# menezesandre/stackrl

Measured on AMD Instinct MI355X. Metric: env steps/sec (batched Stack-v0), higher is better.
Workload: dtype f32

## Files before the change

### stackrl_amd/csrc/settle.hip

```cpp
#include "srl_device.h"
#include "srl_kernels.h"
#include "stage.h"

#ifdef SRL_DIAG_JITTER
__device__ __forceinline__ void srl_jitter_sync() {
  unsigned t = (unsigned)__builtin_readcyclecounter() * 2654435761u + (threadIdx.x >> 6) * 40503u;
  t = __builtin_amdgcn_readfirstlane(t);
  const int n = (t >> 13) & 15;
  for (int i = 0; i < n; ++i) __builtin_amdgcn_s_sleep(16);
  __builtin_amdgcn_fence(__ATOMIC_RELEASE, "workgroup");
  __builtin_amdgcn_s_barrier();
  __builtin_amdgcn_fence(__ATOMIC_ACQUIRE, "workgroup");
  t = t * 1664525u + 1013904223u;
  const int m = (t >> 13) & 15;
  for (int i = 0; i < m; ++i) __builtin_amdgcn_s_sleep(16);
}
#define __syncthreads() srl_jitter_sync()
#endif

template <int T, int PP> struct Variant;

__device__ __forceinline__ int pair_word(int p) {
  int j = (int)((1.0f + sqrtf(1.0f + 8.0f * (float)p)) * 0.5f);
  while (j * (j - 1) / 2 > p) --j;
// ... 416 lines not shown
  const f2 d2 = F2(imp, imp);
#pragma unroll
  for (int c = 0; c < 3; ++c) { u.a[c] = fma2(r.ua[c], d2, u.a[c]); u.b[c] = fma2(r.ub[c], d2, u.b[c]); }
}

__device__ __forceinline__ float contact_target(const DevParams& P, float dist) {
  float inv_dt = 1.0f / P.c.sim_time_step;
  float pen = dist + P.c.linear_slop;
  return pen > 0.0f ? -(pen * inv_dt) : -((pen * P.c.erp) * inv_dt);
}

struct Point {
  PRow n, t1, t2;
  float target, in, i1, i2, ima, imb, mu;
  int a, b;
  int colour;
  int idx;
  bool valid;
};

struct GRow { v3 ca, aa; float rk, k; };
struct GPoint {
  GRow n, t1, t2;
  float target, in, i1, i2, ima, mu;
  int a, idx;
  bool valid;
};

__device__ __forceinline__ GRow make_grow(v3 d, v3 ra, float ima, const m3& Ia) {
  GRow r;
  r.ca = cross(ra, d);
  r.aa = mmul(Ia, r.ca);
  const float k = ima + dot(cross(r.aa, ra), d);
  r.rk = 1.0f / k;
  r.k = k;
  return r;
}

template <int AXIS, int SGN>
__device__ __forceinline__ void grow_solve(const GRow& r, float ima, v3& v, v3& w, float target, float& acc, float lo,
                                           float hi, float& res) {
  float& va = AXIS == 0 ? v.x : AXIS == 1 ? v.y : v.z;
  const float vrel = fmaf(r.ca.x, w.x, fmaf(r.ca.y, w.y, fmaf(r.ca.z, w.z, SGN < 0 ? -va : va)));
  float dl = fmaf(-vrel, r.rk, target * r.rk);
  const float na = __builtin_amdgcn_fmed3f(acc + dl, lo, hi);
  dl = na - acc;
  acc = na;
  res = fmaxf(res, fabsf(dl * r.k));
  va = fmaf(SGN < 0 ? -ima : ima, dl, va);
  w = madd(w, r.aa, dl);
}

template <int AXIS, int SGN>
__device__ __forceinline__ void grow_apply(const GRow& r, float ima, v3& v, v3& w, float imp) {
  float& va = AXIS == 0 ? v.x : AXIS == 1 ? v.y : v.z;
  va = fmaf(SGN < 0 ? -ima : ima, imp, va);
  w = madd(w, r.aa, imp);
}

__device__ __forceinline__ GPoint make_ground_point(const Lds& L, int b, int i) {
  const DevParams& P = *L.P;
  GPoint p;
  p.valid = false; p.a = b; p.idx = i;
  p.in = 0.0f; p.i1 = 0.0f; p.i2 = 0.0f; p.target = 0.0f; p.ima = 0.0f; p.mu = 0.0f;
  const float* g = L.GM(b);
  if (i >= __float_as_int(g[0])) return p;
  p.valid = true;
  p.ima = L.BC(b)[0];
  p.mu = P.c.friction_rock * P.c.friction_ground;
  const m3 Ia = ldm(L.IW(b));
  const int vid = __float_as_int(g[SRL_GM_VID + i]);
  const v3 pw = ld3(L.WV(b) + 3 * vid);
  const v3 ra = V(pw.x, pw.y, pw.z - P.c.collision_margin) - ld3(L.X(b));
  v3 n = V(0.0f, 0.0f, 1.0f), t1, t2;
  plane_space(n, t1, t2);
  p.n = make_grow(n, ra, p.ima, Ia);
  p.t1 = make_grow(t1, ra, p.ima, Ia);
  p.t2 = make_grow(t2, ra, p.ima, Ia);
  p.target = contact_target(P, g[SRL_GM_DIST + i]);
  p.in = g[SRL_GM_IN + i]; p.i1 = g[SRL_GM_T1 + i]; p.i2 = g[SRL_GM_T2 + i];
  return p;
}

template <bool WARM>
__device__ __forceinline__ void ground_turn(const Lds& L, GPoint& p, float& res) {
  const float ws = L.P->c.warmstart;
  v3 v, w;
  ldvw(L, p.a, v, w);
  if (WARM) {
    p.in = p.in * ws; p.i1 = p.i1 * ws; p.i2 = p.i2 * ws;
    grow_apply<2, 1>(p.n, p.ima, v, w, p.in);
    grow_apply<1, -1>(p.t1, p.ima, v, w, p.i1);
    grow_apply<0, 1>(p.t2, p.ima, v, w, p.i2);
  } else {
    grow_solve<2, 1>(p.n, p.ima, v, w, p.target, p.in, 0.0f, 1e30f, res);
    const float lim = p.mu * p.in;
    grow_solve<1, -1>(p.t1, p.ima, v, w, 0.0f, p.i1, -lim, lim, res);
    grow_solve<0, 1>(p.t2, p.ima, v, w, 0.0f, p.i2, -lim, lim, res);
  }
  stvw(L, p.a, v, w);
}

#define SRL_CG_WORDS 28
struct GBody {
  float acc[SRL_GMAXP][3];
  float ima;
  int np, b;
  float* pvw;
  const float4* rec;
};

__device__ __forceinline__ float4* cg_rec(const Lds& L, int b, int i) {
  return (float4*)L.WV(0) + (SRL_CG_WORDS / 4) * (SRL_GMAXP * b + i);
}
__device__ __forceinline__ void cg_store(const Lds& L, const GPoint& p) {
  float4* r = cg_rec(L, p.a, p.idx);
  r[0] = make_float4(p.n.ca.x, p.n.ca.y, p.n.ca.z, p.n.rk);
  r[1] = make_float4(p.n.aa.x, p.n.aa.y, p.n.aa.z, p.target * p.n.rk);
  r[2] = make_float4(p.t1.ca.x, p.t1.ca.y, p.t1.ca.z, p.t1.rk);
  r[3] = make_float4(p.t1.aa.x, p.t1.aa.y, p.t1.aa.z, p.n.k);
  r[4] = make_float4(p.t2.ca.x, p.t2.ca.y, p.t2.ca.z, p.t2.rk);
  r[5] = make_float4(p.t2.aa.x, p.t2.aa.y, p.t2.aa.z, p.t1.k);
  r[6] = make_float4(p.t2.k, p.mu, 0.0f * p.t1.rk, 0.0f * p.t2.rk);
}

template <int AXIS, int SGN>
__device__ __forceinline__ void grow_solve_t(v3 ca, v3 aa, float rk, float k, float ima, v3& v, v3& w, float trk, float& acc,
                                             float lo, float hi, float& res) {
  float& va = AXIS == 0 ? v.x : AXIS == 1 ? v.y : v.z;
  const float vrel = fmaf(ca.x, w.x, fmaf(ca.y, w.y, fmaf(ca.z, w.z, SGN < 0 ? -va : va)));
  float dl = fmaf(-vrel, rk, trk);
  const float na = __builtin_amdgcn_fmed3f(acc + dl, lo, hi);
  dl = na - acc;
  acc = na;
  res = fmaxf(res, fabsf(dl * k));
  va = fmaf(SGN < 0 ? -ima : ima, dl, va);
  w = madd(w, aa, dl);
}

struct GRec { f4 q[7]; };

template <bool WARM>
__device__ __forceinline__ void ground_point(const GRec& R, GBody& gb, int i, float ws, v3& v, v3& w, float& res) {
  const f4 q0 = R.q[0], q1 = R.q[1], q2 = R.q[2], q3 = R.q[3], q4 = R.q[4], q5 = R.q[5], q6 = R.q[6];
  if (WARM) {
    gb.acc[i][0] = gb.acc[i][0] * ws; gb.acc[i][1] = gb.acc[i][1] * ws; gb.acc[i][2] = gb.acc[i][2] * ws;
    GRow g; g.rk = 0.0f; g.k = 0.0f;
    g.ca = V(q0.x, q0.y, q0.z); g.aa = V(q1.x, q1.y, q1.z); grow_apply<2, 1>(g, gb.ima, v, w, gb.acc[i][0]);
    g.ca = V(q2.x, q2.y, q2.z); g.aa = V(q3.x, q3.y, q3.z); grow_apply<1, -1>(g, gb.ima, v, w, gb.acc[i][1]);
    g.ca = V(q4.x, q4.y, q4.z); g.aa = V(q5.x, q5.y, q5.z); grow_apply<0, 1>(g, gb.ima, v, w, gb.acc[i][2]);
  } else {
    grow_solve_t<2, 1>(V(q0.x, q0.y, q0.z), V(q1.x, q1.y, q1.z), q0.w, q3.w, gb.ima, v, w, q1.w, gb.acc[i][0], 0.0f, 1e30f, res);
    const float lim = q6.y * gb.acc[i][0];
    grow_solve_t<1, -1>(V(q2.x, q2.y, q2.z), V(q3.x, q3.y, q3.z), q2.w, q5.w, gb.ima, v, w, q6.z, gb.acc[i][1], -lim, lim, res);
    grow_solve_t<0, 1>(V(q4.x, q4.y, q4.z), V(q5.x, q5.y, q5.z), q4.w, q6.x, gb.ima, v, w, q6.w, gb.acc[i][2], -lim, lim, res);
  }
}

__device__ __forceinline__ GRec cg_load(const float4* rec, int i) {
  GRec R;
#pragma unroll
  for (int k = 0; k < 7; ++k) { const float4 t = rec[7 * i + k]; R.q[k].x = t.x; R.q[k].y = t.y; R.q[k].z = t.z; R.q[k].w = t.w; }
  return R;
}

template <int I>
__device__ __forceinline__ void cg_request(unsigned a, GRec& R, float& tie) {
  asm volatile(
      "ds_read_b128 %0, %8 offset:%9\n\tds_read_b128 %1, %8 offset:%10\n\tds_read_b128 %2, %8 offset:%11\n\t"
      "ds_read_b128 %3, %8 offset:%12\n\tds_read_b128 %4, %8 offset:%13\n\tds_read_b128 %5, %8 offset:%14\n\t"
      "ds_read_b128 %6, %8 offset:%15"
      : "=&v"(R.q[0]), "=&v"(R.q[1]), "=&v"(R.q[2]), "=&v"(R.q[3]), "=&v"(R.q[4]), "=&v"(R.q[5]), "=&v"(R.q[6]), "+v"(tie)
      : "v"(a), "n"(112 * I), "n"(112 * I + 16), "n"(112 * I + 32), "n"(112 * I + 48), "n"(112 * I + 64), "n"(112 * I + 80),
        "n"(112 * I + 96));
}
__device__ __forceinline__ void cg_request_first(unsigned avw, unsigned a, f4& a0, f2& a1, GRec& R) {
  asm volatile(
      "ds_read_b128 %0, %9\n\tds_read_b64 %1, %9 offset:16\n\t"
      "ds_read_b128 %2, %10\n\tds_read_b128 %3, %10 offset:16\n\tds_read_b128 %4, %10 offset:32\n\t"
      "ds_read_b128 %5, %10 offset:48\n\tds_read_b128 %6, %10 offset:64\n\tds_read_b128 %7, %10 offset:80\n\t"
      "ds_read_b128 %8, %10 offset:96"
      : "=&v"(a0), "=&v"(a1), "=&v"(R.q[0]), "=&v"(R.q[1]), "=&v"(R.q[2]), "=&v"(R.q[3]), "=&v"(R.q[4]), "=&v"(R.q[5]), "=&v"(R.q[6])
      : "v"(avw), "v"(a));
}
__device__ __forceinline__ void cg_arrive_first(f4& a0, f2& a1, GRec& R) {
  asm volatile("s_waitcnt lgkmcnt(7)"
               : "+v"(a0), "+v"(a1), "+v"(R.q[0]), "+v"(R.q[1]), "+v"(R.q[2]), "+v"(R.q[3]), "+v"(R.q[4]), "+v"(R.q[5]), "+v"(R.q[6]));
}
template <int LEFT>
__device__ __forceinline__ void cg_arrive(GRec& R, float& tie) {
  asm volatile("s_waitcnt lgkmcnt(%8)"
               : "+v"(R.q[0]), "+v"(R.q[1]), "+v"(R.q[2]), "+v"(R.q[3]), "+v"(R.q[4]), "+v"(R.q[5]), "+v"(R.q[6]), "+v"(tie)
               : "n"(LEFT));
}

template <bool WARM, bool AHEAD, bool KEEP>
__device__ __forceinline__ void ground_body(GBody& gb, float ws, v3& v, v3& w, float& res) {
  static_assert(SRL_CG_WORDS == 28, "cg_request reads seven float4 per record");
  const float4* rec = gb.rec;
  static_assert(SRL_GMAXP == 4, "four nested guards below");
  if (!AHEAD) {
    if (!KEEP) {
      const float4 a0 = *(const float4*)gb.pvw;
      const float2 a1 = *(const float2*)(gb.pvw + 4);
      v = V(a0.x, a0.z, a1.x); w = V(a0.y, a0.w, a1.y);
    }
    ground_point<WARM>(cg_load(rec, 0), gb, 0, ws, v, w, res);
    if (gb.np > 1) {
      ground_point<WARM>(cg_load(rec, 1), gb, 1, ws, v, w, res);
      if (gb.np > 2) {
        ground_point<WARM>(cg_load(rec, 2), gb, 2, ws, v, w, res);
        if (gb.np > 3) ground_point<WARM>(cg_load(rec, 3), gb, 3, ws, v, w, res);
      }
    }
  } else {
    const unsigned ra = (unsigned)(size_t)rec;
    GRec r0, r1, r2, r3;
    if (!KEEP) {
      f4 a0; f2 a1;
      float none = 0.0f;
      cg_request_first((unsigned)(size_t)gb.pvw, ra, a0, a1, r0);
      cg_request<1>(ra, r1, none);
      cg_arrive_first(a0, a1, r0);
      v = V(a0.x, a0.z, a1.x); w = V(a0.y, a0.w, a1.y);
    } else {
      cg_request<0>(ra, r0, w.z);
      cg_request<1>(ra, r1, w.z);
      cg_arrive<7>(r0, w.z);
    }
    ground_point<WARM>(r0, gb, 0, ws, v, w, res);
    cg_arrive<0>(r1, w.x);
    if (gb.np > 1) {
      cg_request<2>(ra, r2, w.z);
      ground_point<WARM>(r1, gb, 1, ws, v, w, res);
      cg_arrive<0>(r2, w.x);
      if (gb.np > 2) {
        cg_request<3>(ra, r3, w.z);
        ground_point<WARM>(r2, gb, 2, ws, v, w, res);
        cg_arrive<0>(r3, w.x);
        if (gb.np > 3) ground_point<WARM>(r3, gb, 3, ws, v, w, res);
      }
    }
  }
  if (!KEEP) { *(float4*)gb.pvw = make_float4(v.x, w.x, v.y, w.y); *(float2*)(gb.pvw + 4) = make_float2(v.z, w.z); }
}

__device__ __forceinline__ Point make_pair_point(const Lds& L, int sl, int i) {
  const DevParams& P = *L.P;
  Point p;
  p.valid = false; p.a = 0; p.b = 0; p.colour = 0; p.idx = i;
  p.in = 0.0f; p.i1 = 0.0f; p.i2 = 0.0f; p.target = 0.0f; p.ima = 0.0f; p.imb = 0.0f; p.mu = 0.0f;
  if (sl >= P.NS) return p;
  const int pid = L.POS()[sl];
  if (pid < 0) return p;
  const float* mp = L.MAN(sl);
  if (i >= __float_as_int(mp[0])) return p;
  p.valid = true;
  L.pair(pid, p.a, p.b);
  p.colour = L.COL()[sl];
  p.ima = L.BC(p.a)[0]; p.imb = L.BC(p.b)[0];
  p.mu = P.c.friction_rock * P.c.friction_rock;
  const float* q = mp + 4 + SRL_MP_WORDS * i;
  const m3 Ra = ldm(L.R(p.a)), Rb = ldm(L.R(p.b));
  const m3 Ia = ldm(L.IW(p.a)), Ib = ldm(L.IW(p.b));
  const v3 ra = mmul(Ra, ld3(q));
  const v3 rb = mmul(Rb, ld3(q + 3));
  v3 n = ld3(q + 6), t1, t2;
  plane_space(n, t1, t2);
  p.n = pack_row(make_row<true>(n, ra, rb, p.ima, Ia, p.imb, Ib), p.ima, p.imb);
  p.t1 = pack_row(make_row<true>(t1, ra, rb, p.ima, Ia, p.imb, Ib), p.ima, p.imb);
  p.t2 = pack_row(make_row<true>(t2, ra, rb, p.ima, Ia, p.imb, Ib), p.ima, p.imb);
  p.target = contact_target(P, q[9]);
  p.in = q[10]; p.i1 = q[11]; p.i2 = q[12];
  return p;
}

template <bool WARM>
__device__ __forceinline__ void point_turn(const Lds& L, Point& p, float& res) {
  const float ws = L.P->c.warmstart;
  Vel2 u;
  float* const pa = L.VW(p.a);
  float* const pb = L.VW(p.b);
  {
    const float4 a0 = *(const float4*)pa, b0 = *(const float4*)pb;
    const float2 a1 = *(const float2*)(pa + 4), b1 = *(const float2*)(pb + 4);
    u.a[0] = F2(a0.x, a0.y); u.a[1] = F2(a0.z, a0.w); u.a[2] = F2(a1.x, a1.y);
    u.b[0] = F2(b0.x, b0.y); u.b[1] = F2(b0.z, b0.w); u.b[2] = F2(b1.x, b1.y);
  }
  if (WARM) {
    p.in = p.in * ws; p.i1 = p.i1 * ws; p.i2 = p.i2 * ws;
    prow_apply(p.n, u, p.in);
    prow_apply(p.t1, u, p.i1);
    prow_apply(p.t2, u, p.i2);
  } else {
    prow_solve(p.n, u, p.target, p.in, 0.0f, 1e30f, res);
    const float lim = p.mu * p.in;
    prow_solve(p.t1, u, 0.0f, p.i1, -lim, lim, res);
    prow_solve(p.t2, u, 0.0f, p.i2, -lim, lim, res);
  }
  *(float4*)pa = make_float4(u.a[0].x, u.a[0].y, u.a[1].x, u.a[1].y); *(float2*)(pa + 4) = make_float2(u.a[2].x, u.a[2].y);
  *(float4*)pb = make_float4(u.b[0].x, u.b[0].y, u.b[1].x, u.b[1].y); *(float2*)(pb + 4) = make_float2(u.b[2].x, u.b[2].y);
}

template <bool WARM, int T, int PP, bool SOLO>
__device__ __forceinline__ bool solver_sweep(const Lds& L, GPoint& gp, GBody& gb, Point (&pp)[PP], int ncol, int gslot,
                                             const int (&pslot)[PP], int gsweep, const unsigned long long (&cm)[2]) {
  typedef Variant<T, PP> VA;
  static_assert(!SOLO || VA::SOLO, "a solo sweep in a variant that has none");
  float res = 0.0f;
  constexpr unsigned long long T0 = 0x1111111111111111ull;
  if (!VA::GROUND_BODY) {
    const unsigned long long gm = __ballot(gslot >= 0);
#pragma unroll
    for (int i = 0; i < SRL_GMAXP; ++i) {
      const unsigned long long t = gm & (T0 << i);
      if (t == 0) break;
      if (__builtin_amdgcn_inverse_ballot_w64(t)) ground_turn<WARM>(L, gp, res);
      __builtin_amdgcn_wave_barrier();
    }
  } else {
    v3 v, w;
    if (gb.np > 0) ground_body<WARM, !WARM && VA::GROUND_AHEAD, false>(gb, L.P->c.warmstart, v, w, res);
    __builtin_amdgcn_wave_barrier();
  }
  int c0 = 0;
  if (SOLO) {
#pragma unroll
    for (int c = 0; c < 2; ++c) {
      if (c >= ncol) break;
#pragma unroll
      for (int i = 0; i < 4; ++i) {
        const unsigned long long t = cm[c] & (T0 << i);
        if (t == 0) break;
        if (__builtin_amdgcn_inverse_ballot_w64(t)) point_turn<WARM>(L, pp[0], res);
        __builtin_amdgcn_wave_barrier();
      }
    }
    c0 = 2;
  }
#pragma unroll 1
  for (int c = c0; c < ncol; ++c) {
    if (!SOLO) __syncthreads();
    unsigned long long mc[PP];
#pragma unroll
    for (int r = 0; r < PP; ++r) mc[r] = __ballot((pslot[r] >> 2) == c);
#pragma unroll
    for (int i = 0; i < 4; ++i) {
      unsigned long long any = 0;
#pragma unroll
      for (int r = 0; r < PP; ++r) any |= mc[r] & (T0 << i);
      if (any == 0) break;
#pragma unroll
      for (int r = 0; r < PP; ++r)
        if (__builtin_amdgcn_inverse_ballot_w64(mc[r] & (T0 << i))) point_turn<WARM>(L, pp[r], res);
      __builtin_amdgcn_wave_barrier();
    }
  }
  if (SOLO) return WARM ? true : __ballot(res * res > L.P->c.residual_threshold) != 0ull;
  int* word = L.MISC() + M_RES0 + (gsweep & 1);
  if (!WARM) {
    if (__ballot(res * res > L.P->c.residual_threshold) != 0ull && (threadIdx.x & 63) == 0) *word = gsweep;
  }
  __syncthreads();
  return WARM ? true : *word == gsweep;
}

#ifdef SRL_STAMPS
#define STAMP(k) do { if (tid == 0) { long long _t = wall_clock64(); L.P->hdr[blockIdx.x].stamps[k] += _t - _t0; _t0 = _t; } } while (0)
#else
#define STAMP(k)
#endif

template <int T, int PP>
__device__ __forceinline__ void substep(const Lds& L, int nb, int tid, int& gsweep) {
  typedef Variant<T, PP> VA;
  const DevParams& P = *L.P;
  if (PP >= 2) asm volatile("" : "+v"(tid));
#ifdef SRL_STAMPS
  long long _t0 = wall_clock64();
#endif
  int* misc = L.MISC();
  if (tid < nb) body_frame(L, tid);
  if (tid == 0) { misc[M_FLAGS] = 0; misc[M_SOLO] = 1; }
  __syncthreads();
  STAMP(0);
  for (int it = tid; it < nb * P.VS; it += T) {
    const int b = it / P.VS, k = it - b * P.VS;
    if (k < __float_as_int(L.BC(b)[5])) {
      const m3 R = ldm(L.R(b));
      v3 lv;
      if (P.S_LV >= 0) lv = ld3(L.LV(b) + 3 * k);
      else { const float4 g4 = P.mv[__float_as_int(L.BC(b)[6]) + k]; lv = V(g4.x, g4.y, g4.z); }
      st3(L.WV(b) + 3 * k, mmul_add(R, lv, ld3(L.X(b))));
    }
  }
  __syncthreads();
  STAMP(1);
  for (int b = tid >> 4; b < nb; b += T >> 4) body_bounds_ground(L, b, tid & 15);
  __syncthreads();
  STAMP(2);
  const int npair = nb * (nb - 1) / 2;
  int fl = 0;
  for (int pid = tid; pid < npair; pid += T) {
    int i, j; L.pair(pid, i, j);
    v3 ai = ld3(L.AMIN(i)), bi = ld3(L.AMAX(i)), aj = ld3(L.AMIN(j)), bj = ld3(L.AMAX(j));
    bool ov = ai.x <= bj.x && aj.x <= bi.x && ai.y <= bj.y && aj.y <= bi.y && ai.z <= bj.z && aj.z <= bi.z;
    int sl = L.SOP()[pid];
    if (!ov && sl >= 0) { L.SOP()[pid] = -1; L.POS()[sl] = -1; fl |= 1; }
    if (ov && sl < 0) fl |= 2;
  }
  if (fl) atomicOr(&misc[M_FLAGS], fl);
  __syncthreads();
  const int flags = misc[M_FLAGS], ncol0 = misc[M_NCOL];
  if (flags || ncol0 < 0) {
    __syncthreads();
    if (tid == 0) {
      if (flags & 2) {
        for (int pid = 0; pid < npair; ++pid) {
          if (L.SOP()[pid] >= 0) continue;
          int i, j; L.pair(pid, i, j);
          v3 ai = ld3(L.AMIN(i)), bi = ld3(L.AMAX(i)), aj = ld3(L.AMIN(j)), bj = ld3(L.AMAX(j));
          bool ov = ai.x <= bj.x && aj.x <= bi.x && ai.y <= bj.y && aj.y <= bi.y && ai.z <= bj.z && aj.z <= bi.z;
          if (!ov) continue;
          int sl = -1;
          for (int k = 0; k < P.NS; ++k) if (L.POS()[k] < 0) { sl = k; break; }
          if (sl < 0) { misc[M_STATUS] |= SRL_ST_PAIR_OVERFLOW; atomicOr(P.flags, 4); continue; }
          L.SOP()[pid] = sl; L.POS()[sl] = pid;
          float* mp = L.MAN(sl);
          mp[0] = __int_as_float(0);
          mp[56] = __int_as_float(0);
          st3(mp + 1, ld3(L.X(i)) - ld3(L.X(j)));
        }
      }
      uint64_t* used = (uint64_t*)(L.sm + P.BLOB + P.S_USED);
      for (int b = 0; b < SRL_MAX_BODIES; ++b) used[b] = 0;
      int nc = 0;
      for (int sl = 0; sl < P.NS; ++sl) {
        int pid = L.POS()[sl];
        if (pid < 0) continue;
        int i, j; L.pair(pid, i, j);
        uint64_t u = used[i] | used[j];
        int c = __ffsll((long long)~u) - 1;
        L.COL()[sl] = c;
        used[i] |= (uint64_t)1 << c;
        used[j] |= (uint64_t)1 << c;
        if (c + 1 > nc) nc = c + 1;
      }
      misc[M_NCOL] = nc;
    }
    __syncthreads();
  }
  const int ncol = misc[M_NCOL];
  STAMP(3);
  {
    constexpr int G = VA::GJK_GROUP;
    const int gl = tid & (G - 1);
    for (int sl = tid / G; sl < P.NS; sl += T / G)
      if (L.POS()[sl] >= 0) narrowphase_slot<G>(L, sl, gl);
  }
  __syncthreads();
  STAMP(4);
  {
    GPoint gp = make_ground_point(L, tid / SRL_GMAXP, tid % SRL_GMAXP);
    if (tid / SRL_GMAXP >= nb) gp.valid = false;
    Point pp[PP];
#pragma unroll
    for (int r = 0; r < PP; ++r) pp[r] = make_pair_point(L, (tid + r * T) >> 2, tid & 3);
    {
      bool mine = gp.valid;
#pragma unroll
      for (int r = 0; r < PP; ++r) mine |= pp[r].valid;
      if (tid >= 64 && __ballot(mine) != 0ull && (tid & 63) == 0) misc[M_SOLO] = 0;
    }
    __syncthreads();
    GBody gb;
    gb.np = 0; gb.b = 0; gb.ima = 0.0f;
    gb.pvw = L.VW(0); gb.rec = cg_rec(L, 0, 0);
#pragma unroll
    for (int i = 0; i < SRL_GMAXP; ++i) { gb.acc[i][0] = 0.0f; gb.acc[i][1] = 0.0f; gb.acc[i][2] = 0.0f; }
    constexpr bool GB = VA::GROUND_BODY, GA = VA::GROUND_AHEAD;
    if (GB) {
    if (gp.valid) cg_store(L, gp);
    if (tid < nb) {
      const float* g = L.GM(tid);
      gb.b = tid; gb.np = __float_as_int(g[0]); gb.ima = L.BC(tid)[0];
      gb.pvw = L.VW(tid); gb.rec = cg_rec(L, tid, 0);
#pragma unroll
      for (int i = 0; i < SRL_GMAXP; ++i)
        if (i < gb.np) { gb.acc[i][0] = g[SRL_GM_IN + i]; gb.acc[i][1] = g[SRL_GM_T1 + i]; gb.acc[i][2] = g[SRL_GM_T2 + i]; }
    }
    __syncthreads();
    }
    STAMP(5);
    const bool solo = VA::SOLO && misc[M_SOLO] != 0;
    const int gslot = gp.valid ? gp.idx : -1;
    unsigned long long cm[2];
    cm[0] = __ballot(pp[0].valid && pp[0].colour == 0); cm[1] = __ballot(pp[0].valid && pp[0].colour == 1);
    int pslot[PP];
#pragma unroll
    for (int r = 0; r < PP; ++r) pslot[r] = pp[r].valid ? 4 * pp[r].colour + pp[r].idx : -1;
    if (solo) {
      int done = 0;
      if (tid < 64) {
        bool anyp = false;
#pragma unroll
        for (int r = 0; r < PP; ++r) anyp |= pp[r].valid;
        const bool ground_only = GB && __ballot(anyp) == 0ull;
        if (ground_only) {
          v3 v = V(0.0f, 0.0f, 0.0f), w = V(0.0f, 0.0f, 0.0f);
          if (gb.np > 0) {
            const float4 a0 = *(const float4*)gb.pvw;
            const float2 a1 = *(const float2*)(gb.pvw + 4);
            v = V(a0.x, a0.z, a1.x); w = V(a0.y, a0.w, a1.y);
            float res = 0.0f;
            ground_body<true, false, true>(gb, P.c.warmstart, v, w, res);
          }
          for (int it = 0; it < P.c.solver_iterations; ++it) {
            done++;
            float res = 0.0f;
            if (gb.np > 0) ground_body<false, GA, true>(gb, P.c.warmstart, v, w, res);
            if (__ballot(res * res > P.c.residual_threshold) == 0ull) break;
          }
          if (gb.np > 0) { *(float4*)gb.pvw = make_float4(v.x, w.x, v.y, w.y); *(float2*)(gb.pvw + 4) = make_float2(v.z, w.z); }
        } else {
          solver_sweep<true, T, PP, VA::SOLO>(L, gp, gb, pp, ncol, gslot, pslot, 0, cm);
          for (int it = 0; it < P.c.solver_iterations; ++it) {
            done++;
            if (!solver_sweep<false, T, PP, VA::SOLO>(L, gp, gb, pp, ncol, gslot, pslot, 0, cm)) break;
          }
        }
        if (tid == 0) misc[M_CNT] = done;
      }
      __syncthreads();
      gsweep += misc[M_CNT];
    } else {
      solver_sweep<true, T, PP, false>(L, gp, gb, pp, ncol, gslot, pslot, 0, cm);
      for (int it = 0; it < P.c.solver_iterations; ++it) {
        gsweep++;
        if (!solver_sweep<false, T, PP, false>(L, gp, gb, pp, ncol, gslot, pslot, gsweep, cm)) break;
      }
    }
#ifdef SRL_STAMPS
    if (tid == 0) {
      EnvHdr* hh = &L.P->hdr[blockIdx.x];
      bool anyp = false;
      for (int r = 0; r < PP; ++r) anyp |= pp[r].valid;
      {
        int bl[SRL_MAX_BODIES]; for (int b = 0; b < SRL_MAX_BODIES; ++b) bl[b] = 0;
        int lmax = 0, sumt = 0;
        for (int c = 0; c < ncol; ++c) {
          int mx = 0;
          for (int sl = 0; sl < P.NS; ++sl) {
            const int pid = L.POS()[sl];
            if (pid < 0 || L.COL()[sl] != c) continue;
            const int np = __float_as_int(L.MAN(sl)[0]);
            if (np <= 0) continue;
            int a, b; L.pair(pid, a, b);
            const int st = bl[a] > bl[b] ? bl[a] : bl[b];
            bl[a] = st + np; bl[b] = st + np;
            if (st + np > lmax) lmax = st + np;
            if (np > mx) mx = np;
          }
          sumt += mx;
        }
        hh->diag[4] += sumt; hh->diag[5] += lmax;
      }
      hh->diag[0] += 1; hh->diag[1] += (__ballot(anyp) == 0ull); hh->diag[2] += ncol; hh->diag[3] += solo ? misc[M_CNT] : 0;
    }
#endif
    if (!GB) {
      if (gp.valid) { float* g = L.GM(gp.a); g[SRL_GM_IN + gp.idx] = gp.in; g[SRL_GM_T1 + gp.idx] = gp.i1; g[SRL_GM_T2 + gp.idx] = gp.i2; }
    } else if (gb.np > 0) {
      float* g = L.GM(gb.b);
#pragma unroll
      for (int i = 0; i < SRL_GMAXP; ++i)
        if (i < gb.np) { g[SRL_GM_IN + i] = gb.acc[i][0]; g[SRL_GM_T1 + i] = gb.acc[i][1]; g[SRL_GM_T2 + i] = gb.acc[i][2]; }
    }
#pragma unroll
    for (int r = 0; r < PP; ++r)
      if (pp[r].valid) {
        float* q = L.MAN((tid + r * T) >> 2) + 4 + SRL_MP_WORDS * pp[r].idx;
        q[10] = pp[r].in; q[11] = pp[r].i1; q[12] = pp[r].i2;
      }
  }
  STAMP(6);
  const float dt = P.c.sim_time_step;
  if (tid < nb) {
    const int b = tid;
    v3 v, w;
    ldvw(L, b, v, w);
    st3(L.X(b), madd(ld3(L.X(b)), v, dt));
    float* Q = L.Q(b);
    q4 q; q.x = Q[0]; q.y = Q[1]; q.z = Q[2]; q.w = Q[3];
    float hx = 0.5f * dt;
    q4 dq;
    dq.x = hx * ((w.x * q.w + w.y * q.z) - w.z * q.y);
    dq.y = hx * ((w.y * q.w + w.z * q.x) - w.x * q.z);
    dq.z = hx * ((w.z * q.w + w.x * q.y) - w.y * q.x);
    dq.w = hx * (-((w.x * q.x + w.y * q.y) + w.z * q.z));
    q.x += dq.x; q.y += dq.y; q.z += dq.z; q.w += dq.w;
    float inv = 1.0f / sqrtf((q.x * q.x + q.y * q.y) + (q.z * q.z + q.w * q.w));
    Q[0] = q.x * inv; Q[1] = q.y * inv; Q[2] = q.z * inv; Q[3] = q.w * inv;
  }
  __syncthreads();
  STAMP(7);
}

__device__ __forceinline__ bool sim_stop(const Lds& L, int nb, int tid) {
  int* misc = L.MISC();
  bool moving = false;
  if (tid < nb) {
    v3 v = ldv(L, tid);
    moving = sqrtf(dot(v, v)) > L.P->c.velocity_threshold;
  }
  if (tid < 64) {
    const unsigned long long m = __ballot(moving);
    if (tid == 0) misc[M_MOVING] = m != 0ull;
  }
  __syncthreads();
  const int any = misc[M_MOVING];
  __syncthreads();
  return !any;
}

__device__ __forceinline__ int newest_contacts(const Lds& L, int nb, int tid, int T) {
  int* misc = L.MISC();
  if (tid == 0) misc[M_CNT] = __float_as_int(L.GM(nb - 1)[0]);
  __syncthreads();
  int n = 0;
  for (int sl = tid; sl < L.P->NS; sl += T) {
    int pid = L.POS()[sl];
    int pi_ = -1, pj_ = -1;
    if (pid >= 0) L.pair(pid, pi_, pj_);
    if (pid >= 0 && (pi_ == nb - 1 || pj_ == nb - 1)) n += __float_as_int(L.MAN(sl)[0]);
  }
  if (n) atomicAdd(&misc[M_CNT], n);
  __syncthreads();
  int r = misc[M_CNT];
  __syncthreads();
  return r;
}

__device__ __forceinline__ MeshHdr stage_mesh_hdr(const MeshHdr* __restrict__ mh, int m) {
  MeshHdr r;
  r.vo = __builtin_amdgcn_readfirstlane(mh[m].vo); r.nv = __builtin_amdgcn_readfirstlane(mh[m].nv);
  r.to = __builtin_amdgcn_readfirstlane(mh[m].to); r.nt = __builtin_amdgcn_readfirstlane(mh[m].nt);
  r.eo = __builtin_amdgcn_readfirstlane(mh[m].eo); r.ne = __builtin_amdgcn_readfirstlane(mh[m].ne);
  r.inv_mass = 0.0f; r.iix = 0.0f; r.iiy = 0.0f; r.iiz = 0.0f; r.radius = 0.0f; r.cx = 0.0f; r.cy = 0.0f; r.cz = 0.0f;
  return r;
}

template <int T>
__device__ __attribute__((noinline)) void stage_tail(const DevParams* __restrict__ Pp, float4* __restrict__ stage, int e, int nb) {
  const DevParams& P = *Pp;
  extern __shared__ __attribute__((aligned(16))) float sm[];
  const int tid = threadIdx.x;
  const int wave = __builtin_amdgcn_readfirstlane(tid >> 6), lane = tid & 63;
  StageLds& S = ((StageLds*)(sm + P.BLOB))[wave];
  StageArgs A;
  A.mp = P.mp; A.mt = P.mt; A.me = P.me; A.mv = P.mv; A.px = P.px; A.inv_px = P.inv_px; A.res = P.c.overhead_res;
  const int slots = P.c.episode_length;
  const float* X = sm + P.OFF_X;
  const float* Q = sm + P.OFF_Q;
  const int* MESH = (const int*)(sm + P.OFF_MESH);
  float4* rec0 = stage + (size_t)e * slots * SRL_STAGE_STRIDE;
  int b = wave;
  if (b >= nb) return;
  MeshHdr mh = stage_mesh_hdr(P.mh, __builtin_amdgcn_readfirstlane(MESH[b]));
  StageLoads g = stage_request(A, mh, lane);
  for (;;) {
    const int bn = b + T / 64;
    const bool more = bn < nb;
    MeshHdr mh_n = mh;
    StageLoads g_n = g;
    if (more) { mh_n = stage_mesh_hdr(P.mh, __builtin_amdgcn_readfirstlane(MESH[bn])); g_n = stage_request(A, mh_n, lane); }
    const float* qq = Q + 4 * b;
    q4 q; q.x = qq[0]; q.y = qq[1]; q.z = qq[2]; q.w = qq[3];
    stage_compute(A, S, rec0 + (size_t)b * SRL_STAGE_STRIDE, ld3(X + 4 * b), q, mh, g, lane);
    __builtin_amdgcn_wave_barrier();
    if (!more) break;
    mh = mh_n; g = g_n; b = bn;
  }
}

template <int T, int PP>
__device__ __forceinline__ void step_body(const DevParams* __restrict__ Pp, const int64_t* __restrict__ action,
                                          int force_reset, const int32_t* __restrict__ order, float4* __restrict__ stage) {
  const DevParams& P = *Pp;
  extern __shared__ __attribute__((aligned(16))) float sm[];
  const int e = order ? order[blockIdx.x] : (int)blockIdx.x, tid = threadIdx.x;
  Lds L; L.init(sm, Pp);
  int* misc = L.MISC();
  EnvHdr* h = &P.hdr[e];
  float* gblob = P.blob + (size_t)e * P.BLOB;
#ifdef SRL_STAMPS
  if ((threadIdx.x & 63) == 0 && threadIdx.x < 128)
    h->hwid[threadIdx.x >> 6] = (long long)__builtin_amdgcn_s_getreg((31 << 11) | 4) | ((long long)__builtin_amdgcn_s_getreg((31 << 11) | 20) << 32);
#endif

  if (tid == 0) {
    int mode;
    if (force_reset < 0) {
      mode = h->nb > 0 ? 4 : 3;
      misc[M_NB] = h->nb;
      misc[M_NCOL] = h->ncolour;
      misc[M_STATUS] = h->status;
      misc[M_RES0] = -1; misc[M_RES1] = -1;
    } else if (!force_reset && action[e] == (int64_t)SRL_ACTION_HOLD) {
      mode = 3;
    } else if (force_reset || h->done) {
      env_reset(P, h, e);
      mode = 1;
    } else {
      int64_t a = action[e];
      int oi = 0, slot = 0;
      if (P.n_slots > 1 && a >= 0) {
        const int nvalid = P.c.ordering_freedom ? h->list_pos * P.n_orient : P.n_orient;
        slot = (int)(a / (int64_t)P.A);
        a = slot < nvalid ? a % (int64_t)P.A : -1;
        oi = slot % P.n_orient;
      }
      misc[M_ORIENT] = oi;
      if (a < 0 || a >= (int64_t)P.A) {
        h->status |= SRL_ST_BAD_ACTION;
        atomicOr(P.flags, 1);
        mode = 2;
      } else {
        h->status &= ~SRL_ST_BAD_ACTION;
        mode = 0;
        misc[M_U] = (int)(a / P.AW);
        misc[M_V] = (int)(a % P.AW);
        int next = -1, placed = h->pending;
        if (P.c.ordering_freedom) {
          const int rk = slot / P.n_orient;
          placed = h->ids[rk];
          for (int k = rk; k + 1 < h->list_pos; ++k) h->ids[k] = h->ids[k + 1];
          h->list_pos -= 1;
          if (h->list_pos == 0) h->done = 1;
          else next = h->ids[0];
        } else if (h->list_pos < P.c.episode_length) next = h->ids[h->list_pos++];
        else h->done = 1;
        misc[M_NEXT] = next;
        misc[M_NB] = h->nb;
        misc[M_PENDING] = placed;
        misc[M_NCOL] = h->ncolour;
        misc[M_STATUS] = h->status;
        misc[M_ZMAX] = (int)f2o(-1e30f);
        misc[M_RES0] = -1; misc[M_RES1] = -1;
      }
    }
    h->mode = mode;
    misc[M_MODE] = mode;
  }
  __syncthreads();
  const int mode = misc[M_MODE];
  if (mode == 1) {
    int* gi = (int*)gblob;
    for (int k = tid; k < P.NP; k += T) gi[P.OFF_SOP + k] = -1;
    for (int k = tid; k < P.NS; k += T) gi[P.OFF_POS + k] = -1;
    return;
  }
  if (mode == 2 || mode == 3) return;

  for (int k = tid; k < P.BLOB; k += T) sm[k] = gblob[k];
  for (int k = tid; k < P.NP; k += T) L.PAIR()[k] = pair_word(k);
  __syncthreads();

  const int u = misc[M_U], v = misc[M_V], pending = misc[M_PENDING];
  int nb = misc[M_NB];
  if (mode == 0) {
    const int res = P.c.overhead_res, r = P.c.object_res;
    const float* Hm = P.H + (size_t)e * res * res;
    const float* Om = P.objmap + ((size_t)pending * P.n_orient + misc[M_ORIENT]) * r * r;
    uint32_t best = f2o(-1e30f);
    for (int k = tid; k < r * r; k += T) {
      int i = k / r, j = k % r;
      float o = Om[k];
      if (o > 1e-4f) {
        uint32_t s = f2o(Hm[(u + i) * res + (v + j)] + o);
        best = s > best ? s : best;
      }
    }
    atomicMax((uint32_t*)&misc[M_ZMAX], best);
  }
  __syncthreads();
  if (tid == 0 && mode == 0) {
    float z = o2f((uint32_t)misc[M_ZMAX]);
    float half = ((float)P.c.object_res * P.px) * 0.5f;
    v3 pos = V((float)u * P.px + half, (float)v * P.px + half, z - half);
    const MeshHdr mh = P.mh[pending];
    int b = nb;
    L.MESH()[b] = pending;
    if (P.n_orient == 1) {
      st3(L.X(b), P.c.place_at_com ? pos : pos + V(mh.cx, mh.cy, mh.cz));
      L.Q(b)[0] = 0.0f; L.Q(b)[1] = 0.0f; L.Q(b)[2] = 0.0f; L.Q(b)[3] = 1.0f;
    } else {
      const float* oq = P.orient_q[misc[M_ORIENT]];
      q4 q; q.x = oq[0]; q.y = oq[1]; q.z = oq[2]; q.w = oq[3];
      st3(L.X(b), P.c.place_at_com ? pos : pos + mmul(quat_to_mat(q), V(mh.cx, mh.cy, mh.cz)));
      L.Q(b)[0] = q.x; L.Q(b)[1] = q.y; L.Q(b)[2] = q.z; L.Q(b)[3] = q.w;
    }
    stvw(L, b, V(0, 0, 0), V(0, 0, 0));
    L.GM(b)[0] = __int_as_float(0);
  }
  if (mode == 0) nb += 1;
  __syncthreads();
  for (int b = tid; b < nb; b += T) {
    int m = L.MESH()[b];
    const MeshHdr mh = P.mh[m];
    float* bc = L.BC(b);
    bc[0] = mh.inv_mass; bc[1] = mh.iix; bc[2] = mh.iiy; bc[3] = mh.iiz; bc[4] = mh.radius;
    bc[5] = __int_as_float(mh.nv); bc[6] = __int_as_float(mh.vo); bc[7] = __int_as_float(m);
  }
  __syncthreads();
  if (P.S_LV >= 0)
  for (int it = tid; it < nb * P.VS; it += T) {
    const int b = it / P.VS, k = it - b * P.VS;
    const float* bc = L.BC(b);
    if (k < __float_as_int(bc[5])) {
      float4 lv = P.mv[__float_as_int(bc[6]) + k];
      st3(L.LV(b) + 3 * k, V(lv.x, lv.y, lv.z));
    }
  }
  __syncthreads();

  enum { PH_PLACE = 0, PH_SMOOTH = 1, PH_ENTER = 2, PH_SETTLE = 3 };
  int counter = 0, phase = PH_PLACE, s_a = 0;
  int gsweep = 0;
  bool diverged = false;
  if (mode == 4) {
    for (int k = 0; k < -force_reset; ++k) substep<T, PP>(L, nb, tid, gsweep);
    for (int k = tid; k < P.BLOB; k += T) gblob[k] = sm[k];
    if (tid == 0) { h->ncolour = misc[M_NCOL]; h->status = misc[M_STATUS]; h->sweeps = gsweep; }
    return;
  }
  for (;;) {
    if (phase == PH_SMOOTH) {
      if (tid == 0) stvw(L, nb - 1, V(0, 0, 0), V(0, 0, 0));
      __syncthreads();
    }
    substep<T, PP>(L, nb, tid, gsweep);
    counter++;
    if (phase != PH_PLACE && counter > P.max_substeps) diverged = true;
    if (phase == PH_PLACE) phase = P.c.smooth_placing ? PH_SMOOTH : PH_ENTER;
    if (phase == PH_SMOOTH) {
      bool leave = diverged;
      if (!leave) {
        const bool drop = newest_contacts(L, nb, tid, T) >= 3;
        const bool stop = sim_stop(L, nb, tid);
        leave = drop || stop;
      }
      if (leave) phase = PH_ENTER;
    }
    if (phase == PH_ENTER) {
      if (tid == 0 && !diverged) {
        st3(L.PX(nb - 1), ld3(L.X(nb - 1)));
        for (int k = 0; k < 4; ++k) L.PQ(nb - 1)[k] = L.Q(nb - 1)[k];
      }
      s_a = counter;
      phase = PH_SETTLE;
    }
    if (phase == PH_SETTLE && (diverged || sim_stop(L, nb, tid))) break;
  }
  __syncthreads();

  for (int k = tid; k < P.BLOB; k += T) gblob[k] = sm[k];
  if (tid == 0) {
    h->nb = nb;
    h->pending = misc[M_NEXT];
    h->ncolour = misc[M_NCOL];
    h->substeps[0] = s_a;
    h->substeps[1] = counter - s_a;
    h->sweeps = gsweep;
    int st = misc[M_STATUS] | (diverged ? SRL_ST_DIVERGED : 0);
    h->status = st;
    if (diverged) atomicOr(P.flags, 2);
  }

  if (stage != nullptr) stage_tail<T>(Pp, stage, e, nb);
}

template <int T, int PP>
struct Variant {
  static constexpr int GJK_GROUP = T == 128 && PP == 1 ? 32 : 16;
  static constexpr bool GROUND_BODY = !(T == 256 && PP == 1);
  static constexpr bool GROUND_AHEAD = T == 128 && PP == 1;
  static constexpr bool SOLO = PP == 1;
};

extern "C" __global__ void __launch_bounds__(128, 2) srl_k_step(const DevParams* __restrict__ Pp,
    const int64_t* __restrict__ action, int force_reset, const int32_t* __restrict__ order, float4* __restrict__ stage) {
  step_body<128, 1>(Pp, action, force_reset, order, stage);
}
extern "C" __global__ void __launch_bounds__(256, 3) srl_k_step_pp1(const DevParams* __restrict__ Pp,
    const int64_t* __restrict__ action, int force_reset, const int32_t* __restrict__ order, float4* __restrict__ stage) {
  step_body<256, 1>(Pp, action, force_reset, order, stage);
}
extern "C" __global__ void __launch_bounds__(256, 2) srl_k_step_pp2(const DevParams* __restrict__ Pp,
    const int64_t* __restrict__ action, int force_reset, const int32_t* __restrict__ order, float4* __restrict__ stage) {
  step_body<256, 2>(Pp, action, force_reset, order, stage);
}

extern "C" __global__ void __launch_bounds__(128, 2) srl_k_step_t128(const DevParams* __restrict__ Pp,
    const int64_t* __restrict__ action, int force_reset, const int32_t* __restrict__ order, float4* __restrict__ stage) {
  step_body<128, 2>(Pp, action, force_reset, order, stage);
}

extern "C" __global__ void __launch_bounds__(64) srl_k_order_keys(const DevParams* __restrict__ Pp,
    const int64_t* __restrict__ action, unsigned long long* __restrict__ keys) {
  const DevParams& P = *Pp;
  const int e = blockIdx.x, lane = threadIdx.x;
  const EnvHdr* h = &P.hdr[e];
  float z = -1.0f;
  int64_t a = action[e];
  if (a != (int64_t)SRL_ACTION_HOLD && !h->done && a >= 0) {
    int slot = 0, mesh = h->pending, nvalid = 1;
    if (P.n_slots > 1) {
      nvalid = P.c.ordering_freedom ? h->list_pos * P.n_orient : P.n_orient;
      slot = (int)(a / (int64_t)P.A);
      a = a % (int64_t)P.A;
      if (P.c.ordering_freedom && slot < nvalid) mesh = h->ids[slot / P.n_orient];
    }
    if (slot < nvalid && a < (int64_t)P.A && mesh >= 0) {
      const int res = P.c.overhead_res, r = P.c.object_res;
      const int u = (int)(a / P.AW), v = (int)(a % P.AW);
      const float* Hm = P.H + (size_t)e * res * res;
      const float* Om = P.objmap + ((size_t)mesh * P.n_orient + slot % P.n_orient) * r * r;
      float best = 0.0f;
      for (int k = lane; k < r * r; k += 64) {
        const float o = Om[k];
        if (o > 1e-4f) best = fmaxf(best, Hm[(u + k / r) * res + (v + k % r)] + o);
      }
      for (int s = 32; s >= 1; s >>= 1) best = fmaxf(best, __shfl_xor(best, s));
      z = best;
    }
  }
  if (lane == 0) keys[e] = ((unsigned long long)(z < 0.0f ? 0xffffffffu : ~__float_as_uint(z)) << 32) | (unsigned)e;
}

extern "C" __global__ void __launch_bounds__(1024) srl_k_order_sort(const unsigned long long* __restrict__ keys, int n, int np2,
                                                                    int32_t* __restrict__ order) {
  extern __shared__ __attribute__((aligned(16))) unsigned long long sk[];
  const int tid = threadIdx.x;
  for (int i = tid; i < np2; i += 1024) sk[i] = i < n ? keys[i] : ~0ull;
  __syncthreads();
  for (int k = 2; k <= np2; k <<= 1)
    for (int j = k >> 1; j >= 1; j >>= 1) {
      for (int t = tid; t < (np2 >> 1); t += 1024) {
        const int i = ((t & ~(j - 1)) << 1) | (t & (j - 1)), p = i | j;
        const unsigned long long a = sk[i], b = sk[p];
        const bool up = (i & k) == 0;
        if ((a > b) == up) { sk[i] = b; sk[p] = a; }
      }
      __syncthreads();
    }
  for (int i = tid; i < n; i += 1024) order[i] = (int32_t)(unsigned)(sk[i] & 0xffffffffull);
}

extern "C" __global__ void srl_k_sample(DevParams P, int64_t* __restrict__ action) {
  int i = blockIdx.x * blockDim.x + threadIdx.x;
  if (i >= P.c.n_envs) return;
  uint32_t key = P.seed + (uint32_t)P.c.env_index_offset + (uint32_t)i;
  int nvalid = P.n_orient;
  if (P.c.ordering_freedom) { const int left = P.hdr[i].list_pos; nvalid *= left > 0 ? left : 1; }
  action[i] = (int64_t)srl_rng_below(srl_rng(key, P.sample_counter, SRL_STREAM_ACTION, 0), (uint32_t)(P.A * nvalid));
}

extern "C" __global__ void srl_k_contacts(DevParams P, float* __restrict__ max_pen, int32_t* __restrict__ n_points) {
  int e = blockIdx.x * blockDim.x + threadIdx.x;
  if (e >= P.c.n_envs) return;
  const float* gb = P.blob + (size_t)e * P.BLOB;
  const int* gi = (const int*)gb;
  int nb = P.hdr[e].nb;
  float mp = 0.0f; int np = 0;
  for (int b = 0; b < nb; ++b) {
    const float* g = gb + P.OFF_GM + SRL_GM_WORDS * b;
    int n = __float_as_int(g[0]);
    for (int k = 0; k < n; ++k) { np++; if (-g[SRL_GM_DIST + k] > mp) mp = -g[SRL_GM_DIST + k]; }
  }
  for (int sl = 0; sl < P.NS; ++sl) {
    if (gi[P.OFF_POS + sl] < 0) continue;
    const float* m = gb + P.OFF_MAN + SRL_MAN_WORDS * sl;
    int n = __float_as_int(m[0]);
    for (int k = 0; k < n; ++k) { np++; float d = m[4 + SRL_MP_WORDS * k + 9]; if (-d > mp) mp = -d; }
  }
  max_pen[e] = mp; n_points[e] = np;
}
```

Measured before the change: 99200.

## Split pair contact rows across lane pairs with DPP quad reduction

For the 128-thread single-point variant, each contact pair slot is now handled by four lanes. Each lane owns one body side and two contact points, and keeps precomputed Jacobian and inverse-mass rows in registers. Relative velocity is reduced across the two sides with a DPP swap, and each lane updates only its own body's velocity. The goal is to remove serialized per-point turns and the repeated LDS reads of both bodies. The cost is higher register pressure and extra setup work per substep.

```diff
diff --git a/stackrl_amd/csrc/settle.hip b/stackrl_amd/csrc/settle.hip
--- a/stackrl_amd/csrc/settle.hip
+++ b/stackrl_amd/csrc/settle.hip
@@ -742,9 +742,161 @@
   *(float4*)pb = make_float4(u.b[0].x, u.b[0].y, u.b[1].x, u.b[1].y); *(float2*)(pb + 4) = make_float2(u.b[2].x, u.b[2].y);
 }
 
+struct HRow { f2 k[3], u[3]; float rk, kk; };
+struct HSet { HRow n, t1, t2; float trk, in, i1, i2; };
+struct PSplit {
+  HSet s0, s1;
+  float* pvw;
+  int np;
+  int colour;
+  float mu;
+};
+
+__device__ __forceinline__ float quad_partner(float x) {
+  return __int_as_float(__builtin_amdgcn_update_dpp(0, __float_as_int(x), 0xB1, 0xf, 0xf, true));
+}
+
+__device__ __forceinline__ HRow make_hrow(v3 d, v3 r, float im, const m3& I, bool side) {
+  HRow h;
+  const v3 c = cross(r, d);
+  const v3 a = mmul(I, c);
+  const float part = im + dot(cross(a, r), d);
+  const float k = part + quad_partner(part);
+  const v3 dm = d * (side ? -im : im);
+  h.k[0] = side ? F2(-d.x, -c.x) : F2(d.x, c.x); h.k[1] = side ? F2(-d.y, -c.y) : F2(d.y, c.y); h.k[2] = side ? F2(-d.z, -c.z) : F2(d.z, c.z);
+  h.u[0] = F2(dm.x, side ? -a.x : a.x); h.u[1] = F2(dm.y, side ? -a.y : a.y); h.u[2] = F2(dm.z, side ? -a.z : a.z);
+  h.rk = 1.0f / k; h.kk = k;
+  return h;
+}
+
+__device__ __forceinline__ HSet make_hset(const Lds& L, const float* mp, int i, int np, int body, bool side) {
+  const DevParams& P = *L.P;
+  HSet s;
+  s.trk = 0.0f; s.in = 0.0f; s.i1 = 0.0f; s.i2 = 0.0f;
+  if (i >= np) {
+    HRow z;
+    z.k[0] = z.k[1] = z.k[2] = z.u[0] = z.u[1] = z.u[2] = F2(0.0f, 0.0f); z.rk = 0.0f; z.kk = 0.0f;
+    s.n = z; s.t1 = z; s.t2 = z;
+    return s;
+  }
+  const float im = L.BC(body)[0];
+  const float* q = mp + 4 + SRL_MP_WORDS * i;
+  const v3 r = mmul(ldm(L.R(body)), ld3(q + (side ? 3 : 0)));
+  const m3 I = ldm(L.IW(body));
+  v3 n = ld3(q + 6), t1, t2;
+  plane_space(n, t1, t2);
+  s.n = make_hrow(n, r, im, I, side);
+  s.t1 = make_hrow(t1, r, im, I, side);
+  s.t2 = make_hrow(t2, r, im, I, side);
+  s.trk = contact_target(P, q[9]) * s.n.rk;
+  s.in = q[10]; s.i1 = q[11]; s.i2 = q[12];
+  return s;
+}
+
+__device__ __forceinline__ int slot_points(const Lds& L, int sl) {
+  if (sl >= L.P->NS || L.POS()[sl] < 0) return 0;
+  return __float_as_int(L.MAN(sl)[0]);
+}
+
+__device__ __forceinline__ PSplit make_pair_split(const Lds& L, int tid) {
+  const DevParams& P = *L.P;
+  const int sl = tid >> 2, h = (tid >> 1) & 1;
+  const bool side = tid & 1;
+  PSplit p;
+  p.np = 0; p.colour = 0; p.pvw = L.VW(0);
+  p.mu = P.c.friction_rock * P.c.friction_rock;
+  int body = 0;
+  const float* mp = L.MAN(0);
+  if (sl < P.NS) {
+    const int pid = L.POS()[sl];
+    if (pid >= 0) {
+      int a, b; L.pair(pid, a, b);
+      body = side ? b : a;
+      mp = L.MAN(sl);
+      p.np = __float_as_int(mp[0]);
+      p.colour = L.COL()[sl];
+      p.pvw = L.VW(body);
+    }
+  }
+  p.s0 = make_hset(L, mp, 2 * h, p.np, body, side);
+  p.s1 = make_hset(L, mp, 2 * h + 1, p.np, body, side);
+  return p;
+}
+
+__device__ __forceinline__ void hrow_solve(const HRow& r, f2 (&u)[3], float trk, float& acc, float lo, float hi, float& res) {
+  const f2 s = fma2(r.k[0], u[0], fma2(r.k[1], u[1], r.k[2] * u[2]));
+  float own = s.x + s.y;
+  asm("" : "+v"(own));
+  const float vrel = own + quad_partner(own);
+  float dl = fmaf(-vrel, r.rk, trk);
+  const float na = __builtin_amdgcn_fmed3f(acc + dl, lo, hi);
+  dl = na - acc;
+  acc = na;
+  res = fmaxf(res, fabsf(dl * r.kk));
+  const f2 d2 = F2(dl, dl);
+#pragma unroll
+  for (int c = 0; c < 3; ++c) u[c] = fma2(r.u[c], d2, u[c]);
+}
+
+__device__ __forceinline__ float zero_times(float rk) {
+  float t;
+  asm volatile("v_mul_f32 %0, 0, %1" : "=v"(t) : "v"(rk));
+  return t;
+}
+
+template <bool WARM>
+__device__ __forceinline__ void hset_turn(HSet& s, f2 (&u)[3], float mu, float ws, float& res) {
+  if (WARM) {
+    s.in = s.in * ws; s.i1 = s.i1 * ws; s.i2 = s.i2 * ws;
+    const f2 dn = F2(s.in, s.in), d1 = F2(s.i1, s.i1), d2 = F2(s.i2, s.i2);
+#pragma unroll
+    for (int c = 0; c < 3; ++c) u[c] = fma2(s.n.u[c], dn, u[c]);
+#pragma unroll
+    for (int c = 0; c < 3; ++c) u[c] = fma2(s.t1.u[c], d1, u[c]);
+#pragma unroll
+    for (int c = 0; c < 3; ++c) u[c] = fma2(s.t2.u[c], d2, u[c]);
+  } else {
+    hrow_solve(s.n, u, s.trk, s.in, 0.0f, 1e30f, res);
+    const float lim = mu * s.in;
+    hrow_solve(s.t1, u, zero_times(s.t1.rk), s.i1, -lim, lim, res);
+    hrow_solve(s.t2, u, zero_times(s.t2.rk), s.i2, -lim, lim, res);
+  }
+}
+
+__device__ __forceinline__ void hvel_load(const float* p, f2 (&u)[3]) {
+  const float4 a0 = *(const float4*)p;
+  const float2 a1 = *(const float2*)(p + 4);
+  u[0] = F2(a0.x, a0.y); u[1] = F2(a0.z, a0.w); u[2] = F2(a1.x, a1.y);
+}
+__device__ __forceinline__ void hvel_store(float* p, const f2 (&u)[3]) {
+  *(float4*)p = make_float4(u[0].x, u[0].y, u[1].x, u[1].y); *(float2*)(p + 4) = make_float2(u[2].x, u[2].y);
+}
+
+template <bool WARM>
+__device__ __forceinline__ void pair_phase(PSplit& p, float ws, unsigned long long m1, unsigned long long m2, float& res) {
+  constexpr unsigned long long LO = 0x3333333333333333ull;
+#pragma unroll
+  for (int h = 0; h < 2; ++h) {
+    const unsigned long long t1 = m1 & (LO << (2 * h)), t2 = m2 & (LO << (2 * h));
+    if (t1 == 0) return;
+    if (__builtin_amdgcn_inverse_ballot_w64(t1)) {
+      f2 u[3];
+      hvel_load(p.pvw, u);
+      hset_turn<WARM>(p.s0, u, p.mu, ws, res);
+      if (t2 != 0) {
+        if (__builtin_amdgcn_inverse_ballot_w64(t2)) hset_turn<WARM>(p.s1, u, p.mu, ws, res);
+      }
+      hvel_store(p.pvw, u);
+    }
+    __builtin_amdgcn_wave_barrier();
+    if (t2 == 0) return;
+  }
+}
+
 template <bool WARM, int T, int PP, bool SOLO>
-__device__ __forceinline__ bool solver_sweep(const Lds& L, GPoint& gp, GBody& gb, Point (&pp)[PP], int ncol, int gslot,
-                                             const int (&pslot)[PP], int gsweep, const unsigned long long (&cm)[2]) {
+__device__ __forceinline__ bool solver_sweep(const Lds& L, GPoint& gp, GBody& gb, Point (&pp)[PP], PSplit& sp, int ncol, int gslot,
+                                             const int (&pslot)[PP], int gsweep, const unsigned long long (&cm)[2],
+                                             const unsigned long long (&cm2)[2]) {
   typedef Variant<T, PP> VA;
   static_assert(!SOLO || VA::SOLO, "a solo sweep in a variant that has none");
   float res = 0.0f;
@@ -768,6 +920,9 @@
 #pragma unroll
     for (int c = 0; c < 2; ++c) {
       if (c >= ncol) break;
+      if constexpr (VA::PAIR_SPLIT) {
+        pair_phase<WARM>(sp, L.P->c.warmstart, cm[c], cm2[c], res);
+      } else {
 #pragma unroll
       for (int i = 0; i < 4; ++i) {
         const unsigned long long t = cm[c] & (T0 << i);
@@ -775,12 +930,18 @@
         if (__builtin_amdgcn_inverse_ballot_w64(t)) point_turn<WARM>(L, pp[0], res);
         __builtin_amdgcn_wave_barrier();
       }
+      }
     }
     c0 = 2;
   }
 #pragma unroll 1
   for (int c = c0; c < ncol; ++c) {
     if (!SOLO) __syncthreads();
+    if constexpr (VA::PAIR_SPLIT) {
+      const int h2 = (threadIdx.x >> 1) & 1;
+      const bool mine = sp.colour == c;
+      pair_phase<WARM>(sp, L.P->c.warmstart, __ballot(mine && sp.np > 2 * h2), __ballot(mine && sp.np > 2 * h2 + 1), res);
+    } else {
     unsigned long long mc[PP];
 #pragma unroll
     for (int r = 0; r < PP; ++r) mc[r] = __ballot((pslot[r] >> 2) == c);
@@ -794,6 +955,7 @@
       for (int r = 0; r < PP; ++r)
         if (__builtin_amdgcn_inverse_ballot_w64(mc[r] & (T0 << i))) point_turn<WARM>(L, pp[r], res);
       __builtin_amdgcn_wave_barrier();
+    }
     }
   }
   if (SOLO) return WARM ? true : __ballot(res * res > L.P->c.residual_threshold) != 0ull;
@@ -815,7 +977,7 @@
 __device__ __forceinline__ void substep(const Lds& L, int nb, int tid, int& gsweep) {
   typedef Variant<T, PP> VA;
   const DevParams& P = *L.P;
-  if (PP >= 2) asm volatile("" : "+v"(tid));
+  if (PP >= 2 || VA::PAIR_SPLIT) asm volatile("" : "+v"(tid));
 #ifdef SRL_STAMPS
   long long _t0 = wall_clock64();
 #endif
@@ -904,8 +1066,14 @@
     GPoint gp = make_ground_point(L, tid / SRL_GMAXP, tid % SRL_GMAXP);
     if (tid / SRL_GMAXP >= nb) gp.valid = false;
     Point pp[PP];
+    PSplit sp;
+    if constexpr (VA::PAIR_SPLIT) {
+#pragma unroll
+      for (int r = 0; r < PP; ++r) pp[r].valid = slot_points(L, tid >> 2) > 0;
+    } else {
 #pragma unroll
     for (int r = 0; r < PP; ++r) pp[r] = make_pair_point(L, (tid + r * T) >> 2, tid & 3);
+    }
     {
       bool mine = gp.valid;
 #pragma unroll
@@ -931,14 +1099,25 @@
     }
     __syncthreads();
     }
+    if constexpr (VA::PAIR_SPLIT) sp = make_pair_split(L, tid);
     STAMP(5);
     const bool solo = VA::SOLO && misc[M_SOLO] != 0;
     const int gslot = gp.valid ? gp.idx : -1;
-    unsigned long long cm[2];
+    unsigned long long cm[2], cm2[2] = {0ull, 0ull};
+    int pslot[PP];
+    if constexpr (VA::PAIR_SPLIT) {
+      const int h2 = (tid >> 1) & 1;
+#pragma unroll
+      for (int c = 0; c < 2; ++c) {
+        cm[c] = __ballot(sp.colour == c && sp.np > 2 * h2); cm2[c] = __ballot(sp.colour == c && sp.np > 2 * h2 + 1);
+      }
+#pragma unroll
+      for (int r = 0; r < PP; ++r) pslot[r] = -1;
+    } else {
     cm[0] = __ballot(pp[0].valid && pp[0].colour == 0); cm[1] = __ballot(pp[0].valid && pp[0].colour == 1);
-    int pslot[PP];
 #pragma unroll
     for (int r = 0; r < PP; ++r) pslot[r] = pp[r].valid ? 4 * pp[r].colour + pp[r].idx : -1;
+    }
     if (solo) {
       int done = 0;
       if (tid < 64) {
@@ -963,10 +1142,10 @@
           }
           if (gb.np > 0) { *(float4*)gb.pvw = make_float4(v.x, w.x, v.y, w.y); *(float2*)(gb.pvw + 4) = make_float2(v.z, w.z); }
         } else {
-          solver_sweep<true, T, PP, VA::SOLO>(L, gp, gb, pp, ncol, gslot, pslot, 0, cm);
+          solver_sweep<true, T, PP, VA::SOLO>(L, gp, gb, pp, sp, ncol, gslot, pslot, 0, cm, cm2);
           for (int it = 0; it < P.c.solver_iterations; ++it) {
             done++;
-            if (!solver_sweep<false, T, PP, VA::SOLO>(L, gp, gb, pp, ncol, gslot, pslot, 0, cm)) break;
+            if (!solver_sweep<false, T, PP, VA::SOLO>(L, gp, gb, pp, sp, ncol, gslot, pslot, 0, cm, cm2)) break;
           }
         }
         if (tid == 0) misc[M_CNT] = done;
@@ -974,10 +1153,10 @@
       __syncthreads();
       gsweep += misc[M_CNT];
     } else {
-      solver_sweep<true, T, PP, false>(L, gp, gb, pp, ncol, gslot, pslot, 0, cm);
+      solver_sweep<true, T, PP, false>(L, gp, gb, pp, sp, ncol, gslot, pslot, 0, cm, cm2);
       for (int it = 0; it < P.c.solver_iterations; ++it) {
         gsweep++;
-        if (!solver_sweep<false, T, PP, false>(L, gp, gb, pp, ncol, gslot, pslot, gsweep, cm)) break;
+        if (!solver_sweep<false, T, PP, false>(L, gp, gb, pp, sp, ncol, gslot, pslot, gsweep, cm, cm2)) break;
       }
     }
 #ifdef SRL_STAMPS
@@ -1016,12 +1195,21 @@
       for (int i = 0; i < SRL_GMAXP; ++i)
         if (i < gb.np) { g[SRL_GM_IN + i] = gb.acc[i][0]; g[SRL_GM_T1 + i] = gb.acc[i][1]; g[SRL_GM_T2 + i] = gb.acc[i][2]; }
     }
+    if constexpr (VA::PAIR_SPLIT) {
+      const int i0 = tid & 2;
+      if (!(tid & 1) && sp.np > i0) {
+        float* q = L.MAN(tid >> 2) + 4 + SRL_MP_WORDS * i0;
+        q[10] = sp.s0.in; q[11] = sp.s0.i1; q[12] = sp.s0.i2;
+        if (sp.np > i0 + 1) { q[SRL_MP_WORDS + 10] = sp.s1.in; q[SRL_MP_WORDS + 11] = sp.s1.i1; q[SRL_MP_WORDS + 12] = sp.s1.i2; }
+      }
+    } else {
 #pragma unroll
     for (int r = 0; r < PP; ++r)
       if (pp[r].valid) {
         float* q = L.MAN((tid + r * T) >> 2) + 4 + SRL_MP_WORDS * pp[r].idx;
         q[10] = pp[r].in; q[11] = pp[r].i1; q[12] = pp[r].i2;
       }
+    }
   }
   STAMP(6);
   const float dt = P.c.sim_time_step;
@@ -1326,6 +1514,7 @@
   static constexpr bool GROUND_BODY = !(T == 256 && PP == 1);
   static constexpr bool GROUND_AHEAD = T == 128 && PP == 1;
   static constexpr bool SOLO = PP == 1;
+  static constexpr bool PAIR_SPLIT = T == 128 && PP == 1;
 };
 
 extern "C" __global__ void __launch_bounds__(128, 2) srl_k_step(const DevParams* __restrict__ Pp,
```

Result: faster. 112,300, median of 6 (+13.3%).
